# sarahappleby/VAMP

Measured on AMD Instinct MI355X. Metric: walker-steps/sec (log-posterior evals/sec), higher is better.
Workload: dtype f64

## Files before the change

vamp_amd/csrc/ff_moments.hpp:

```cpp
#pragma once
#include "voigt_math.hpp"

namespace vamp {

constexpr int FFM_NS = 14, FFM_NQ = 27, FFM_QROW = 28;
constexpr int FFM_S = 4 * FFM_QROW;
constexpr int FFM_TILE = FFM_S + 4 * FFM_NS;
constexpr int FFM_C0 = 0 * FFM_QROW + FFM_NQ;
constexpr int FFM_RC = 1 * FFM_QROW + FFM_NQ;
constexpr int FFM_RQ = 2 * FFM_QROW + FFM_NQ;

constexpr double FFM_ULPS = 8.0;
constexpr double FFM_BOUND = 256.0 / 1099511627776.0;
constexpr double FFM_RMAX = 512.0;
VAMP_DEV bool ff_moments_ok(double root_c0, double root_q0, double amax) {
    return fma(amax, root_q0, root_c0) <= FFM_RMAX;
}
VAMP_DEV bool ff_moments_try(double root_c0, double root_q0) {
    return ff_moments_ok(root_c0, root_q0, 0.0) && root_c0 + root_c0 <= FFM_RMAX;
}

}
```

vamp_amd/csrc/vamp_hip.hip:

```cpp
#include <hip/hip_runtime.h>
#include <dlfcn.h>

#include <algorithm>
#include <atomic>
#include <chrono>
#include <cmath>
#include <cstdint>
#include <cstdio>
#include <cstdlib>
#include <cstring>
#include <new>
#include <string>
#include <vector>

#include "../../include/vamp_hip.h"
#include "abi_state.hpp"
#include "draws.hpp"
#include "host_plan.hpp"
#include "map_search.hpp"
#include "voigt_math.hpp"
#include "ff_predicates.hpp"
#include "ff_moments.hpp"

#ifndef VAMP_EARLY_LOADS
#define VAMP_EARLY_LOADS 1
#endif
#ifndef VAMP_BLEND_PASS_LINES
#define VAMP_BLEND_PASS_LINES 4
#endif
#ifndef VAMP_MID_MIN_K
#define VAMP_MID_MIN_K 3
#endif
#ifndef VAMP_MID_MIN_P
#define VAMP_MID_MIN_P 96
#endif
#ifndef VAMP_X_PREFETCH
#define VAMP_X_PREFETCH 0
#endif

#ifndef VAMP_MIN_WAVES
#define VAMP_MIN_WAVES 3
#endif
#ifndef VAMP_EARLY_LNP
#define VAMP_EARLY_LNP 1
#endif
#ifndef VAMP_SR_EARLY
#define VAMP_SR_EARLY 0
#endif
#ifndef VAMP_XCD_MAP
#define VAMP_XCD_MAP 0
#endif
#ifndef VAMP_WIDE_NODES
#define VAMP_WIDE_NODES 1
#endif
#ifndef VAMP_LPT
#define VAMP_LPT 1
#endif
#ifndef VAMP_FLUX_EXP_DROP
#define VAMP_FLUX_EXP_DROP 2
#endif
#ifndef VAMP_FF_R2_M4
#define VAMP_FF_R2_M4 100.0
#define VAMP_FF_R2_M3 300.0
#define VAMP_FF_R2_M2 2000.0
#endif
#ifndef VAMP_F32_FAR_CORE
#define VAMP_F32_FAR_CORE 1
#endif
#ifndef VAMP_CORE_FASTPATH
#define VAMP_CORE_FASTPATH 1
#endif
#ifndef VAMP_MID_NODES
#define VAMP_MID_NODES 1
#endif
#ifndef VAMP_MID_Z2
#define VAMP_MID_Z2 30.25
#endif
#ifndef VAMP_WIDE_MAX
#define VAMP_WIDE_MAX 0.75
#endif
#ifndef VAMP_F32_LEAN_STAGE
#define VAMP_F32_LEAN_STAGE 1
#endif
#ifndef VAMP_TILE_MOMENTS
#define VAMP_TILE_MOMENTS 1
#endif
namespace {

constexpr int KMAX = 16;
constexpr int KMAX_ALL = VAMP_MAX_COMPONENTS;
static_assert(KMAX_ALL >= KMAX && KMAX_ALL < 64, "lane k stages line k; one spare lane for sd");
constexpr int WAVES_PER_BLOCK = 4;
constexpr long long PACK_MIN_WALKERS = 16384;
constexpr int RES_MAX_MOVERS = 128;
#ifndef VAMP_RES_WAVES
#define VAMP_RES_WAVES 8
#endif
constexpr int RES_MAX_WAVES = VAMP_RES_WAVES;
constexpr int BLOCK = 64 * WAVES_PER_BLOCK;
constexpr int DMAX = 4 * KMAX_ALL + 1;
#ifndef VAMP_SPLIT_MAX_WALKERS
#define VAMP_SPLIT_MAX_WALKERS (1ll << 62)
#endif
constexpr long long SPLIT_MAX_WALKERS = VAMP_SPLIT_MAX_WALKERS;

constexpr double C_LIGHT = 2.98e8;
constexpr double SIGMA0 = 0.0263;
constexpr double SQRT_LN2 = 0.83255461115769775635;
constexpr double SQRT_PI = 1.77245385090551602730;
constexpr double FWHM_PER_SIGMA = 2.35482004503094938202;
constexpr double NEG_INF = -__builtin_huge_val();

using vamp::RegionDev;

struct LineRec {
    double c;
    double s;
    double y;
    double amp;
    double pole;
    double hy;
    double xcap;
    double w8, w25;
    double wmid;
};

#ifndef VAMP_PARTS
#define VAMP_PARTS 4
#endif
constexpr int PARTS = VAMP_PARTS;
template <int KCAP, bool OWN_DTAB> struct WalkerLds;
#ifdef VAMP_STAMPS
__device__ unsigned long long g_stamps[2 * 8192];
__device__ unsigned int g_stamp_n;
#define VAMP_STAMP(tag)                                                                          \
    do {                                                                                         \
        if (blockIdx.x == 0 && threadIdx.x == 0) {                                               \
            const unsigned int n_ = g_stamp_n;                                                   \
            if (n_ < 8192) { g_stamps[2 * n_] = (tag); g_stamps[2 * n_ + 1] = __builtin_amdgcn_s_memtime(); g_stamp_n = n_ + 1; } \
        }                                                                                        \
    } while (0)
#define VAMP_STAMP_AFTER(tag, v) do { asm volatile("" :: "v"(v)); VAMP_STAMP(tag); } while (0)
#else
#define VAMP_STAMP(tag) do {} while (0)
#define VAMP_STAMP_AFTER(tag, v) do {} while (0)
#endif
#ifndef VAMP_SPLIT_WAVES
#define VAMP_SPLIT_WAVES 4
#endif
#ifndef VAMP_SPLIT_WAVES_F32
#define VAMP_SPLIT_WAVES_F32 4
#endif
#ifndef VAMP_F32_TABLES
#define VAMP_F32_TABLES 1
#endif
template <int LPW_, int KCAP_, bool TAIL_, int WPB_, bool SPLIT_ = false, bool TABS_ = SPLIT_, bool FF_ = (LPW_ == 64)>
struct Pack {
    static constexpr int LPW = LPW_, KCAP = KCAP_, SUBS = 64 / LPW_;
    static constexpr bool TAIL = TAIL_;
    static constexpr bool SPLIT = SPLIT_;
    static constexpr bool TABS = TABS_;
    static constexpr bool FF = FF_;
    static constexpr int WPB = WPB_;
    static constexpr int THREADS = 64 * WPB_;
    static constexpr int WALKERS_PER_BLOCK = SPLIT_ ? 1 : WPB_ * SUBS;
    static constexpr int LINES_PER_PASS = (SPLIT_ && TABS_ && !FF_ && WPB_ == 1) ? VAMP_BLEND_PASS_LINES : 0;
    static constexpr int TAB_LINES = LINES_PER_PASS > 0 ? LINES_PER_PASS : KCAP_;
    static constexpr bool DTAB_IN_TABLES = SPLIT_ && TABS_ && FF_;
// ... 552 lines not shown
}
template <class real>
__device__ __forceinline__ void ff_series(TileScratch& Sx, const double* __restrict__ dct, int lane, double fs) {
    if (lane < FF_NODES) Sx.coef[lane] = fs;
    __builtin_amdgcn_wave_barrier();
    const double2* mrow = reinterpret_cast<const double2*>(dct) + (lane < FF_ROWS ? lane : FF_ROWS - 1);
    const double2* fv = reinterpret_cast<const double2*>(Sx.coef);
    double a0 = 0.0, a1 = 0.0;
#pragma unroll
    for (int n2 = 0; n2 < FF_NODES / 2; ++n2) {
        const double2 m = mrow[n2 * FF_ROWS], f2 = fv[n2];
        a0 = fma(m.x, f2.x, a0);
        a1 = fma(m.y, f2.y, a1);
    }
    __builtin_amdgcn_wave_barrier();
    if (lane < FF_ROWS) reinterpret_cast<real*>(Sx.coef)[lane] = (real)(a0 + a1);
    __builtin_amdgcn_wave_barrier();
}
template <class LDS, bool GUARD = true>
__device__ __forceinline__ double ff_node_sums(const LDS& L, const unsigned char* farlist, const double* __restrict__ dct,
                                               int lane_, int nfar, double mid, double half, double fs_wide = 0.0) {
    int lane = lane_;
    asm volatile("" : "+v"(lane));
    const int node = lane & (FF_NODES - 1), grp = lane >> 4;
    const double tnode = dct[FF_MAT + node];
    __builtin_amdgcn_wave_barrier();
    const double xnode = fma(half, tnode, mid);
    double Xn[4], yn[4], an[4];
#pragma unroll
    for (int t = 0; t < 4; ++t) {
        const int q = 4 * t + grp;
        const unsigned kf = nfar > 0 ? farlist[q < nfar ? q : nfar - 1] : 0u;
        const LineRec& ln = *reinterpret_cast<const LineRec*>(reinterpret_cast<const char*>(L.line) + __umul24(kf, (unsigned)sizeof(LineRec)));
        Xn[t] = fabs(xnode - ln.c) * ln.s;
        yn[t] = ln.y;
        an[t] = q < nfar ? ln.amp : 0.0;
    }
    double fs = 0.0;
    if (nfar > 0) {
        const double Xa[2] = {Xn[0], Xn[1]}, ya[2] = {yn[0], yn[1]};
        double Ha[2];
        ff_eval2<GUARD>(Xa, ya, Ha, dct + FF_EXP);
        fs = fma(an[0], Ha[0], an[1] * Ha[1]);
    }
    if (nfar > 8) {
        const double Xb[2] = {Xn[2], Xn[3]}, yb[2] = {yn[2], yn[3]};
        double Hb[2];
        ff_eval2<GUARD>(Xb, yb, Hb, dct + FF_EXP);
        fs += fma(an[2], Hb[0], an[3] * Hb[1]);
    }
    fs += fs_wide;
    fs += __hiloint2double(__builtin_amdgcn_ds_bpermute((lane ^ 16) << 2, __double2hiint(fs)),
                           __builtin_amdgcn_ds_bpermute((lane ^ 16) << 2, __double2loint(fs)));
    fs += __hiloint2double(__builtin_amdgcn_ds_bpermute((lane ^ 32) << 2, __double2hiint(fs)),
                           __builtin_amdgcn_ds_bpermute((lane ^ 32) << 2, __double2loint(fs)));
    return fs;
}
template <class LDS, bool GUARD = true>
__device__ __forceinline__ void ff_coefficients(const LDS& L, TileScratch& Sx, const unsigned char* farlist, const double* __restrict__ dct,
                                                int lane, int nfar, double mid, double half, double fs_wide = 0.0) {
    ff_series<double>(Sx, dct, lane, ff_node_sums<LDS, GUARD>(L, farlist, dct, lane, nfar, mid, half, fs_wide));
}
__device__ __forceinline__ void ff_moment_chi(TileScratch& Sx, const double* __restrict__ dct, const double* __restrict__ mt, int lane,
                                              double a, double& chi) {
    const int row = lane < FF_ROWS ? lane : FF_ROWS - 1;
    const int q = row / (FF_DEG + 1), j = row - q * (FF_DEG + 1);
    ff_series<double>(Sx, dct, lane, a);
    const double* Qw = mt + q * vamp::FFM_QROW + j;
    double Qv[FF_DEG + 1];
#pragma unroll
    for (int l = 0; l <= FF_DEG; ++l) Qv[l] = Qw[l];
    const double Sv = mt[vamp::FFM_S + row], c0 = mt[vamp::FFM_C0];
    const double* bq = Sx.coef + q * (FF_DEG + 1);
    double acc0 = Sv + Sv, acc1 = 0.0;
#pragma unroll
    for (int l = 0; l <= FF_DEG; l += 2) {
        acc0 = fma(bq[l], Qv[l], acc0);
        acc1 = fma(bq[l + 1], Qv[l + 1], acc1);
    }
    const double term = Sx.coef[row] * (acc0 + acc1);
    chi += lane < FF_ROWS ? term : lane == FF_ROWS ? c0 : 0.0;
    __builtin_amdgcn_wave_barrier();
}
template <class LDS>
__device__ __forceinline__ double ff_wide_nodes(const LDS& L, const unsigned char* widelist, const double* __restrict__ dct, const double* tab,
                                                int lane, int nwide, double mid, double half) {
    const int node = lane & (FF_NODES - 1), grp = lane >> 4;
    const double xnode = fma(half, dct[FF_MAT + node], mid);
    double fs = 0.0;
    for (int t = 0; 4 * t < nwide; ++t) {
        const int q = 4 * t + grp;
        const int k = widelist[q < nwide ? q : nwide - 1];
        const LineRec& ln = L.line[k];
        const double X = fabs(xnode - ln.c) * ln.s, r2 = fma(X, X, ln.y * ln.y);
        double H;
        if (r2 < vamp::R2_CORE) {
            H = table_eval(tab + k * vamp::TAB_LINE, X);
        } else {
            H = vamp::voigt_jfrac<6>(X, ln.y, r2);
            if (ln.y < vamp::Y_TINY) H += vamp::SQRT_PI * vamp::exp_neg_sq_tab(X, dct + FF_EXP);
        }
        fs = fma(q < nwide ? ln.amp : 0.0, H, fs);
    }
    return fs;
}
template <class real, int T>
__device__ __forceinline__ void ff_horner(const TileScratch& Sx, const real (&u)[T], bool up, real (&tau)[T]) {
    static_assert(T == 4, "one pixel per quarter of the tile");
    real acc[T];
    const real* cq[T];
#pragma unroll
    for (int t = 0; t < T; ++t) {
        const int q = up ? t : T - 1 - t;
        cq[t] = reinterpret_cast<const real*>(Sx.coef) + q * (FF_DEG + 1);
        acc[t] = cq[t][FF_DEG];
    }
#pragma unroll
    for (int j = FF_DEG - 1; j >= 0; --j) {
#pragma unroll
        for (int t = 0; t < T; ++t) acc[t] = fma(acc[t], u[t], cq[t][j]);
    }
#pragma unroll
    for (int t = 0; t < T; ++t) tau[t] += acc[t];
    __builtin_amdgcn_wave_barrier();
}

template <int MODE, class PK, bool TAB, bool WIDE = false, bool GUARD = true>
__device__ __forceinline__ void sweep_range_ff(const RegionDev& R, const typename PK::Lds& L, TileScratch& Sx, const double* __restrict__ dct,
                                               const double* __restrict__ x, const double* __restrict__ f,
                                               const double* __restrict__ wt, const double* __restrict__ ut,
                                               const double2* __restrict__ geo, int lane, int base0, int base1, int stride,
                                               double& chi, const double* tab, unsigned long long wide_all = 0ull,
                                               const double* __restrict__ mom = nullptr) {
    constexpr int T = TPIX;
    static_assert(PK::LPW == 64 && PK::KCAP <= 16, "far-field tiles: one walker per wavefront, <= 16 lines");
    const int K = R.K;
#if VAMP_X_PREFETCH
    double xn[T];
    if (base0 < base1) {
#pragma unroll
        for (int t = 0; t < T; ++t) xn[t] = x[base0 + 64 * t + lane];
    }
#endif
    for (int batch = base0; batch < base1; batch += FF_BATCH * stride) {
    unsigned long long farmasks, widemasks, zonemasks;
    ff_classify_batch<WIDE, false, TAB>(L, Sx, geo, K, lane, batch, base1, stride, (unsigned)wide_all, farmasks, widemasks, zonemasks);
#if VAMP_TILE_MOMENTS && !defined(VAMP_SKIP_FFNODES)
    {
        unsigned long long fm = farmasks, wm = widemasks;
#pragma unroll 1
        for (int j = 0; j < FF_BATCH; ++j, fm >>= KMAX, wm >>= KMAX) {
            const int base = batch + j * stride;
            if (base >= base1) break;
            const unsigned farmask = (unsigned)fm & 0xffffu, widemask = WIDE ? (unsigned)wm & 0xffffu : 0u;
            if ((~(farmask | widemask) & ((1u << K) - 1u)) != 0u) continue;
            const double* mt = mom + (base >> 8) * vamp::FFM_TILE;
            const double root_c0 = mt[vamp::FFM_RC], root_q0 = mt[vamp::FFM_RQ];
            if (!vamp::ff_moments_try(root_c0, root_q0)) continue;
            const double2 tg = geo[base >> 8];
            const double mid = tg.x, half = fabs(tg.y);
            const int nfar = __builtin_popcount(farmask), nwide = __builtin_popcount(widemask);
            const int ln = lane_here();
            double fs_wide = 0.0;
            if constexpr (WIDE) {
                if (nwide > 0) fs_wide = ff_wide_nodes<typename PK::Lds>(L, Sx.widelist[j], dct, tab, ln, nwide, mid, half);
            }
            const double fs = ff_node_sums<typename PK::Lds, GUARD>(L, Sx.farlist[j], dct, ln, nfar, mid, half, fs_wide);
            int eoff = FF_EXP;
            asm volatile("" : "+s"(eoff));
            const double a = -vamp::expm1_taylor_tab(-fs, dct + eoff);
            const double amax = row16_max(fabs(a));
            if (!__builtin_amdgcn_readfirstlane((int)vamp::ff_moments_ok(root_c0, root_q0, amax))) continue;
            ff_moment_chi(Sx, dct, mt, ln, a, chi);
            const unsigned long long field = 0xffffull << (KMAX * j);
            farmasks |= field;
            widemasks |= field;
        }
    }
#endif
#pragma unroll 1
    for (int j = 0; j < FF_BATCH; ++j, farmasks >>= KMAX, widemasks >>= KMAX, zonemasks >>= KMAX) {
        const int base = batch + j * stride;
        if (base >= base1) break;
        double xi[T], tau[T];
#if VAMP_X_PREFETCH
#pragma unroll
        for (int t = 0; t < T; ++t) {
            xi[t] = xn[t];
            tau[t] = 0.0;
        }
        {
            const int nb = base + stride < base1 ? base + stride : base;
#pragma unroll
            for (int t = 0; t < T; ++t) xn[t] = x[nb + 64 * t + lane];
        }
#else
#pragma unroll
        for (int t = 0; t < T; ++t) {
            xi[t] = x[base + 64 * t + lane];
            tau[t] = 0.0;
        }
#endif
        if ((unsigned)farmasks & (unsigned)widemasks & 0xffffu) continue;
        const double2 tg = geo[base >> 8];
        const double mid = tg.x, half = fabs(tg.y);
        const bool up = __double2hiint(tg.y) >= 0;
        const unsigned farmask = (unsigned)farmasks & 0xffffu;
        const int nfar = __builtin_popcount(farmask);
        const unsigned widemask = WIDE ? (unsigned)widemasks & 0xffffu : 0u;
        const int nwide = __builtin_popcount(widemask);
#ifndef VAMP_SKIP_NEAR
        for (unsigned near = ~(farmask | widemask) & ((1u << K) - 1u); near; near &= near - 1u) {
            const int k = __builtin_ctz(near);
            const LineRec ln = L.line[k];
            double X[T], H[T];
#pragma unroll
            for (int t = 0; t < T; ++t) X[t] = fabs(xi[t] - ln.c) * ln.s;
            if (TAB && (((unsigned)zonemasks >> k) & 1u)) {
#pragma unroll
                for (int t = 0; t < T; ++t) H[t] = table_eval(tab + k * vamp::TAB_LINE, X[t]);
            } else {
                tile_voigt<T, TAB>(ln, dtab_row<PK>(L, k), X, H, TAB ? tab + k * vamp::TAB_LINE : nullptr, dct + FF_EXP);
            }
#pragma unroll
            for (int t = 0; t < T; ++t) tau[t] = fma(ln.amp, H[t], tau[t]);
        }
#endif
        double fi[T], wi[T];
        if (nfar + nwide > 0) {
            double u[T];
#pragma unroll
            for (int t = 0; t < T; ++t) u[t] = ut[base + 64 * t + lane];
#ifndef VAMP_SKIP_FFNODES
            double fs_wide = 0.0;
            if constexpr (WIDE) {
                if (nwide > 0) {
                    fs_wide = ff_wide_nodes<typename PK::Lds>(L, Sx.widelist[j], dct, tab, lane, nwide, mid, half);
                }
            }
            ff_coefficients<typename PK::Lds, GUARD>(L, Sx, Sx.farlist[j], dct, lane, nfar, mid, half, fs_wide);
#endif
#if VAMP_EARLY_LOADS
#pragma unroll
            for (int t = 0; t < T; ++t) {
                fi[t] = f[base + 64 * t + lane];
                wi[t] = wt[base + 64 * t + lane];
            }
            __builtin_amdgcn_sched_barrier(0);
#endif
#ifndef VAMP_SKIP_CLENSHAW
            ff_horner<double, T>(Sx, u, up, tau);
#endif
        } else {
#if VAMP_EARLY_LOADS
#pragma unroll
            for (int t = 0; t < T; ++t) {
// ... 214 lines not shown
            tau[t] = 0.0f;
        }
        const double2 tg = geo[base >> 8];
        const double mid = tg.x, half = fabs(tg.y);
        const bool up = __double2hiint(tg.y) >= 0;
        const unsigned farmask = (unsigned)farmasks & 0xffffu;
        const int nfar = __builtin_popcount(farmask);
#ifndef VAMP_SKIP_NEAR
        for (unsigned near = ~farmask & ((1u << K) - 1u); near; near &= near - 1u) {
            const int k = __builtin_ctz(near);
            const float c = L.linef[k][0], sc = L.linef[k][1], y = L.linef[k][2], a = L.linef[k][3];
            float X[T], H[T];
#pragma unroll
            for (int t = 0; t < T; ++t) X[t] = fabsf(xi[t] - c) * sc;
            if constexpr (TAB32) tile_w4_tab<T>(y, X, H, tab32 + k * vamp::TAB32_LINE);
            else tile_w4<T>(y, X, H);
#pragma unroll
            for (int t = 0; t < T; ++t) tau[t] = fmaf(a, H[t], tau[t]);
        }
#endif
        if (nfar > 0) {
            float u[T];
#pragma unroll
            for (int t = 0; t < T; ++t) u[t] = ut[base + 64 * t + lane];
#ifndef VAMP_SKIP_FFNODES
            ff32_coefficients<typename PK::Lds>(L, Sx, Sx.farlist[j], reinterpret_cast<const float*>(dct), lane, nfar, mid, half);
#endif
#ifndef VAMP_SKIP_CLENSHAW
            ff32_horner<T>(Sx, u, up, tau);
#endif
        }
#pragma unroll
        for (int t = 0; t < T; ++t) {
            const int i = base + 64 * t + lane;
#ifdef VAMP_SKIP_EXP
            const float m = 1.0f - tau[t];
#else
            const float m = __expf(-tau[t]);
#endif
            const float r = (f[i] - m) * wt[i];
            chi += (double)r * (double)r;
        }
    }
    }
}

struct PixPtrs {
    const double* x; const double* f; const double* wt;
    const float* xf; const float* ff; const float* wtf;
    const double* u; const float* uf; const double2* geo;
    const double* mom;
};

template <bool F32>
__global__ __launch_bounds__(64 * TPIX) void k_tile_tables(const RegionDev* __restrict__ regions, const double* __restrict__ x,
                                                           const float* __restrict__ xf, double* __restrict__ u, float* __restrict__ uf,
                                                           double2* __restrict__ geo, const double* __restrict__ f = nullptr,
                                                           const double* __restrict__ wt = nullptr, double* __restrict__ mom = nullptr) {
    const RegionDev& R = regions[blockIdx.y];
    const int base = (int)blockIdx.x * (64 * TPIX), i = base + (int)threadIdx.x;
    if (i >= R.P) return;
    const long long g = R.pix_off + i;
    if (base + 64 * TPIX > R.P) {
        if constexpr (F32) uf[g] = 0.0f;
        else u[g] = 0.0;
        return;
    }
    const long long g0 = R.pix_off + base, g1 = g0 + 64 * TPIX - 1;
    const double x_lo = F32 ? (double)xf[g0] : x[g0], x_hi = F32 ? (double)xf[g1] : x[g1];
    const double mid = 0.5 * (x_lo + x_hi), half = 0.5 * fabs(x_hi - x_lo);
    const bool up = x_hi > x_lo;
    const int t = (int)threadIdx.x >> 6, q = up ? t : TPIX - 1 - t;
    double ug = 0.0;
    if constexpr (F32) {
        const float hf = (float)half, mf = (float)mid;
        const float scale = 4.0f * __builtin_amdgcn_rcpf(hf);
        uf[g] = (xf[g] - fmaf(hf, 0.5f * q - 0.75f, mf)) * scale;
    } else {
        const double scale = 4.0 * vamp::rcp_nr(half);
        ug = (x[g] - fma(half, 0.5 * q - 0.75, mid)) * scale;
        u[g] = ug;
    }
    if (threadIdx.x == 0) geo[g0 >> 8] = make_double2(mid, up ? half : -half);
#if VAMP_TILE_MOMENTS
    if constexpr (!F32) {
        __shared__ double part[TPIX][2];
        double* mt = mom + (g0 >> 8) * vamp::FFM_TILE;
        const int lane = (int)threadIdx.x & 63;
        const double w2 = wt[g] * wt[g], d = f[g] - 1.0, w2d = w2 * d;
        double pw = 1.0;
        for (int n = 0; n < vamp::FFM_NQ; ++n) {
            const double sq = wave_sum<64>(w2 * pw);
            if (lane == 0) mt[q * vamp::FFM_QROW + n] = sq;
            if (n == 0 && lane == 0) part[q][0] = sq;
            if (n < vamp::FFM_NS) {
                const double ss = wave_sum<64>(w2d * pw);
                if (lane == 0) mt[vamp::FFM_S + q * vamp::FFM_NS + n] = ss;
            }
            pw *= ug;
        }
        const double c0 = wave_sum<64>(w2d * d);
        if (lane == 0) part[q][1] = c0;
        __syncthreads();
        if (threadIdx.x == 0) {
            const double q0 = (part[0][0] + part[1][0]) + (part[2][0] + part[3][0]);
            const double C0 = (part[0][1] + part[1][1]) + (part[2][1] + part[3][1]);
            mt[vamp::FFM_C0] = C0;
            mt[vamp::FFM_RC] = sqrt(C0);
            mt[vamp::FFM_RQ] = sqrt(q0);
            mt[3 * vamp::FFM_QROW + vamp::FFM_NQ] = 0.0;
        }
    }
#endif
}

template <bool F32, int MODE, class PK, bool TAB = use_tables<F32, MODE, PK>()>
__device__ __forceinline__ void sweep_class(const RegionDev& R, const typename PK::Lds& L, TileScratch& Sx, const double* __restrict__ dct,
                                            const PixPtrs& px, int lane, int base0, int full, int stride, bool tail, double& chi,
                                            const double* tab) {
    constexpr int TPIX = pixels_per_lane<PK>();
    if constexpr (F32) {
        const float* x = px.xf + R.pix_off; const float* f = px.ff + R.pix_off; const float* wt = px.wtf + R.pix_off;
        if constexpr (VAMP_FARFIELD && PK::FF && MODE != VAMP_GAUSS3 && TPIX == 4)
            sweep_range_f32_ff<MODE, PK, use_tables32<F32, MODE, PK>()>(R, L, Sx, dct, x, f, wt, px.uf + R.pix_off, px.geo + (R.pix_off >> 8),
                                                                        lane, base0, full, stride, chi, reinterpret_cast<const float*>(tab));
        else if (TPIX > 1) sweep_range_f32<MODE, PK, TPIX>(R, L, x, f, wt, lane, base0, full, stride, chi);
        if constexpr (PK::TAIL || TPIX == 1)
            if (tail) {
                const int from = TPIX > 1 ? full : 0;
                if constexpr (!PK::FF && TPIX > 1) {
                    const int nt = (R.P - from + PK::LPW - 1) / PK::LPW;
                    if constexpr (TPIX >= 4) { if (nt == 4) sweep_range_f32<MODE, PK, 4>(R, L, x, f, wt, lane, from, from + 1, 1 << 28, chi); }
                    if constexpr (TPIX >= 3) { if (nt == 3) sweep_range_f32<MODE, PK, 3>(R, L, x, f, wt, lane, from, from + 1, 1 << 28, chi); }
                    if (nt == 2) sweep_range_f32<MODE, PK, 2>(R, L, x, f, wt, lane, from, from + 1, 1 << 28, chi);
                    else if (nt == 1) sweep_range_f32<MODE, PK, 1>(R, L, x, f, wt, lane, from, from + 1, 1 << 28, chi);
                } else {
                    sweep_range_f32<MODE, PK, 1>(R, L, x, f, wt, lane, from, R.P, PK::LPW, chi);
                }
            }
    } else {
        const double* x = px.x + R.pix_off; const double* f = px.f + R.pix_off; const double* wt = px.wt + R.pix_off;
        if constexpr (VAMP_FARFIELD && PK::FF && MODE != VAMP_GAUSS3 && TPIX == 4) {
            const double* ut = px.u + R.pix_off;
            const double2* geo = px.geo + (R.pix_off >> 8);
            const double* mom = VAMP_TILE_MOMENTS ? px.mom + (R.pix_off >> 8) * vamp::FFM_TILE : nullptr;
            const int flags = __builtin_amdgcn_readfirstlane((int)(__double_as_longlong(L.theta[4 * PK::KCAP + 2]) & 0x3ffff));
            const bool guard = (flags >> 16) != 0;
            if constexpr (VAMP_WIDE_NODES && TAB) {
                const unsigned long long wide_all = (unsigned long long)(flags & 0xffff);
                if (VAMP_MID_NODES || wide_all) {
                    if (guard) sweep_range_ff<MODE, PK, TAB, true, true>(R, L, Sx, dct, x, f, wt, ut, geo, lane, base0, full, stride, chi, tab, wide_all, mom);
                    else sweep_range_ff<MODE, PK, TAB, true, false>(R, L, Sx, dct, x, f, wt, ut, geo, lane, base0, full, stride, chi, tab, wide_all, mom);
                } else {
                    if (guard) sweep_range_ff<MODE, PK, TAB, false, true>(R, L, Sx, dct, x, f, wt, ut, geo, lane, base0, full, stride, chi, tab, 0ull, mom);
                    else sweep_range_ff<MODE, PK, TAB, false, false>(R, L, Sx, dct, x, f, wt, ut, geo, lane, base0, full, stride, chi, tab, 0ull, mom);
                }
            } else {
                if (guard) sweep_range_ff<MODE, PK, TAB, false, true>(R, L, Sx, dct, x, f, wt, ut, geo, lane, base0, full, stride, chi, tab, 0ull, mom);
                else sweep_range_ff<MODE, PK, TAB, false, false>(R, L, Sx, dct, x, f, wt, ut, geo, lane, base0, full, stride, chi, tab, 0ull, mom);
            }
        } else if (TPIX > 1) sweep_range<MODE, PK, TPIX, TAB>(R, L, x, f, wt, lane, base0, full, stride, chi, tab);
        if constexpr (PK::TAIL || TPIX == 1)
            if (tail) {
                const int from = TPIX > 1 ? full : 0;
                if constexpr (!PK::FF && TPIX > 1) {
                    const int nt = (R.P - from + PK::LPW - 1) / PK::LPW;
                    if constexpr (TPIX >= 4) { if (nt == 4) sweep_range<MODE, PK, 4, TAB>(R, L, x, f, wt, lane, from, from + 1, 1 << 28, chi, tab); }
                    if constexpr (TPIX >= 3) { if (nt == 3) sweep_range<MODE, PK, 3, TAB>(R, L, x, f, wt, lane, from, from + 1, 1 << 28, chi, tab); }
                    if (nt == 2) sweep_range<MODE, PK, 2, TAB>(R, L, x, f, wt, lane, from, from + 1, 1 << 28, chi, tab);
                    else if (nt == 1) sweep_range<MODE, PK, 1, TAB>(R, L, x, f, wt, lane, from, from + 1, 1 << 28, chi, tab);
                } else {
                    sweep_range<MODE, PK, 1, TAB>(R, L, x, f, wt, lane, from, R.P, PK::LPW, chi, tab);
                }
            }
    }
}

template <int MODE, class PK, int T>
__device__ __forceinline__ void blend_chunk(const RegionDev& R, const typename PK::Lds& L, const double* __restrict__ x, int lane,
                                            int base, int k0, int kn, const double* tab, double (&tau)[4]) {
    double xi[T];
#pragma unroll
    for (int t = 0; t < T; ++t) {
        const int i = base + 64 * t + lane;
        xi[t] = x[i < R.P ? i : R.P - 1];
    }
    for (int kk = 0; kk < kn; ++kk) {
        const LineRec ln = L.line[k0 + kk];
        double X[T], H[T];
#pragma unroll
        for (int t = 0; t < T; ++t) X[t] = fabs(xi[t] - ln.c) * ln.s;
        tile_voigt<T, true>(ln, L.dtab[k0 + kk], X, H, tab + kk * vamp::TAB_LINE);
#pragma unroll
        for (int t = 0; t < T; ++t) tau[t] = fma(ln.amp, H[t], tau[t]);
    }
}
template <int MODE, class PK>
__device__ __forceinline__ void blend_chunk_n(const RegionDev& R, const typename PK::Lds& L, const double* __restrict__ x, int lane,
                                              int base, int tn, int k0, int kn, const double* tab, double (&tau)[4]) {
    if (tn >= 4) blend_chunk<MODE, PK, 4>(R, L, x, lane, base, k0, kn, tab, tau);
    else if (tn == 3) blend_chunk<MODE, PK, 3>(R, L, x, lane, base, k0, kn, tab, tau);
    else if (tn == 2) blend_chunk<MODE, PK, 2>(R, L, x, lane, base, k0, kn, tab, tau);
    else if (tn == 1) blend_chunk<MODE, PK, 1>(R, L, x, lane, base, k0, kn, tab, tau);
}
constexpr int BLEND_MAX_PIXELS = 512;
template <int MODE, class PK>
__device__ __forceinline__ double sweep_blend_passes(const RegionDev& R, const typename PK::Lds& L, const PixPtrs& px, int lane,
                                                     double* tab) {
    static_assert(PK::WPB == 1 && PK::LPW == 64, "one wavefront per walker");
    constexpr int LP = PK::LINES_PER_PASS;
    const double* __restrict__ x = px.x + R.pix_off;
    const double* __restrict__ f = px.f + R.pix_off;
    const double* __restrict__ wt = px.wt + R.pix_off;
    const int P = R.P, K = R.K;
    const int nt = (P + 63) >> 6;
    const int tn0 = nt < 4 ? nt : 4, tn1 = nt - tn0;
    double tau0[4] = {0.0, 0.0, 0.0, 0.0}, tau1[4] = {0.0, 0.0, 0.0, 0.0};
    for (int k0 = 0; k0 < K; k0 += LP) {
        const int kn = K - k0 < LP ? K - k0 : LP;
        for (int e = lane; e < kn * vamp::TAB_NI; e += 64) {
            const int kk = e / vamp::TAB_NI, i = e % vamp::TAB_NI, k = k0 + kk;
            vamp::taylor_table_row(i, L.line[k].y, L.dtab[k], L.line[k].pole, L.line[k].hy, tab + kk * vamp::TAB_LINE + i * vamp::TAB_NT);
        }
        group_barrier<PK>();
        blend_chunk_n<MODE, PK>(R, L, x, lane, 0, tn0, k0, kn, tab, tau0);
        if (tn1 > 0) blend_chunk_n<MODE, PK>(R, L, x, lane, 256, tn1, k0, kn, tab, tau1);
        group_barrier<PK>();
    }
// ... 1316 lines not shown
    if (c->comm && c->exchange && c->shard_parts > 1)
        for (int p = 0; p < c->shard_parts; ++p) HIP_TRY(hipStreamWaitEvent(c->stream, c->ev_scatter[p], 0));
    return 0;
}

int free_comm(vamp_ctx* c) {
    if (c->rccl) {
        RcclApi* api = nullptr;
        if (rccl_api(&api) == 0) (void)api->CommDestroy(c->rccl);
        c->rccl = nullptr;
    }
    for (hipEvent_t e : c->ev_kernel) (void)hipEventDestroy(e);
    for (hipEvent_t e : c->ev_scatter) (void)hipEventDestroy(e);
    c->ev_kernel.clear();
    c->ev_scatter.clear();
    if (c->comm_stream) (void)hipStreamDestroy(c->comm_stream);
    c->comm_stream = nullptr;
    vamp::leave_comm(c);
    return 0;
}

}

extern "C" {

long long vampdbg_resident_plan(vamp_ctx* c, int max_classes, long long* rows) {
    if (!c || !rows || max_classes < 0) return fail(VAMP_ERR_ARG, "vampdbg_resident_plan: bad argument");
    if (!c->sampler_ready) return fail(VAMP_ERR_STATE, "vampdbg_resident_plan: call vamp_sampler_init first");
    const long long halfW = c->W / 2;
    const std::vector<LaunchClass>& classes = partition_for(c, halfW);
    for (size_t ci = 0; ci < classes.size() && (int)ci < max_classes; ++ci) {
        const LaunchClass& cl = classes[ci];
        const int shape = launch_shape(c, cl, halfW);
        const int nw = resident_waves_for(c, shape, halfW);
        long long lds = 0;
        VAMP_FOR_MODE_PK(c->f32, c->mode, shape, lds = resident_lds<F32, M, PK>(nw));
        long long* row = rows + 4 * ci;
        row[0] = cl.kind;
        row[1] = nw;
        row[2] = (long long)nw * (shape_walkers_per_block(shape) / shape_waves(shape));
        row[3] = lds;
    }
    return (long long)classes.size();
}

long long vampdbg_launch_plan(vamp_ctx* c, long long movers_per_region, int entry, int region, int max_classes, long long* rows) {
    if (!c || !rows || max_classes < 0 || entry < 0 || entry > 3 || movers_per_region < 1) return fail(VAMP_ERR_ARG, "vampdbg_launch_plan: bad argument");
    if (c->regions_h.empty()) return fail(VAMP_ERR_STATE, "vampdbg_launch_plan: call vamp_set_regions first");
    if (region >= c->n_regions || (entry == 2 && region < 0)) return fail(VAMP_ERR_ARG, "vampdbg_launch_plan: no such region");
    const long long per = entry == 3 ? MAP_MOVERS : movers_per_region;
    const std::vector<LaunchClass>& classes = partition_for(c, per);
    const std::vector<int>& class_of = class_of_for(c, per);
    long long n = 0;
    for (size_t ci = 0; ci < classes.size(); ++ci) {
        const LaunchClass& cl = classes[ci];
        if (region >= 0 && class_of[region] != (int)ci) continue;
        if (n < max_classes) {
            const int shape = launch_shape(c, cl, per);
            long long* row = rows + 5 * n;
            row[0] = cl.kind;
            row[1] = shape;
            row[2] = shape_walkers_per_block(shape);
            row[3] = shape_threads(shape);
            row[4] = (long long)cl.regions.size();
        }
        ++n;
    }
    return n;
}

long long vampdbg_tile_tables(vamp_ctx* c, double* u_out, float* uf_out, double* geo_out) {
    if (!c || !geo_out || !(c->f32 ? (void*)uf_out : (void*)u_out)) return fail(VAMP_ERR_ARG, "vampdbg_tile_tables: bad argument");
    if (c->regions_h.empty()) return fail(VAMP_ERR_STATE, "vampdbg_tile_tables: call vamp_set_regions first");
    if (!c->geo_d) return 0;
    const long long N = c->regions_h.back().pix_off + c->regions_h.back().P;
    const long long slots = N / (64 * TPIX) + 1;
    HIP_TRY(hipStreamSynchronize(c->stream));
    if (c->f32) HIP_TRY(hipMemcpy(uf_out, c->uf_d.get(), N * sizeof(float), hipMemcpyDeviceToHost));
    else HIP_TRY(hipMemcpy(u_out, c->u_d.get(), N * sizeof(double), hipMemcpyDeviceToHost));
    HIP_TRY(hipMemcpy(geo_out, c->geo_d.get(), slots * sizeof(double2), hipMemcpyDeviceToHost));
    return slots;
}

int vamp_version(void) { return VAMP_ABI_VERSION; }

const char* vamp_last_error(void) { return vamp::last_error().c_str(); }

int vamp_device_count(int* n) {
    if (int rc = vamp::check_device_count(n)) return rc;
    HIP_TRY(hipGetDeviceCount(n));
    return VAMP_OK;
}

int vamp_ctx_create(vamp_ctx** out, int device, int dtype, int wofz_kind) {
    if (int rc = vamp::check_ctx_create(out, dtype, wofz_kind)) return rc;
    int ndev = 0;
    HIP_TRY(hipGetDeviceCount(&ndev));
    if (int rc = vamp::check_device(device, ndev)) return rc;
    HIP_TRY(hipSetDevice(device));
    vamp_ctx* c = nullptr;
    if (int rc = vamp::new_ctx(&c, dtype)) return rc;
    c->device = device;
    c->wofz_kind = wofz_kind;
    hipError_t e = hipStreamCreateWithFlags(&c->own_stream, hipStreamNonBlocking);
    if (e != hipSuccess) {
        delete c;
        return fail(VAMP_ERR_HIP, std::string("hipStreamCreate: ") + hipGetErrorString(e));
    }
    c->stream = c->own_stream;
    if (const char* e = getenv("VAMP_CLASS_STREAMS")) c->concurrent_classes = std::atoi(e) != 0;
    if (const char* e = getenv("VAMP_RESIDENT")) c->opt_resident = std::max(0, std::min(2, std::atoi(e)));
    if (const char* e = getenv("VAMP_MAP_DEVICE")) c->opt_map_device = std::atoi(e) != 0;
    *out = c;
    return VAMP_OK;
}

int vamp_ctx_destroy(vamp_ctx* c) {
    if (!c) return VAMP_OK;
    (void)hipSetDevice(c->device);
    (void)hipStreamSynchronize(c->stream);
    if (c->comm_stream) (void)hipStreamSynchronize(c->comm_stream);
    free_comm(c);
    for (hipStream_t st : c->cls_stream) (void)hipStreamDestroy(st);
    for (hipEvent_t e : c->ev_join) (void)hipEventDestroy(e);
    if (c->ev_fork) (void)hipEventDestroy(c->ev_fork);
    if (c->own_stream) (void)hipStreamDestroy(c->own_stream);
    delete c;
    return VAMP_OK;
}

int vamp_ctx_set_stream(vamp_ctx* c, void* hip_stream) {
    if (int rc = vamp::need_ctx(c, "vamp_ctx_set_stream")) return rc;
    HIP_TRY(hipStreamSynchronize(c->stream));
    c->stream = hip_stream ? (hipStream_t)hip_stream : c->own_stream;
    return VAMP_OK;
}

int vamp_ctx_set_stream_default(vamp_ctx* c) {
    if (int rc = vamp::need_ctx(c, "vamp_ctx_set_stream_default")) return rc;
    HIP_TRY(hipStreamSynchronize(c->stream));
    c->stream = nullptr;
    return VAMP_OK;
}

int vamp_ctx_set_packing(vamp_ctx* c, int lanes_per_walker) { return vamp::set_packing(c, lanes_per_walker); }

int vamp_ctx_set_option(vamp_ctx* c, const char* name, int64_t value) {
    if (int rc = vamp::check_option(c, name)) return rc;
    const std::string key(name);
    if (key == "map_device") c->opt_map_device = value != 0;
    else if (key == "resident") c->opt_resident = value < 0 ? 0 : value > 2 ? 2 : (int)value;
    else c->concurrent_classes = value != 0;
    return VAMP_OK;
}

int vamp_ctx_synchronize(vamp_ctx* c) {
    if (int rc = vamp::need_ctx(c, "vamp_ctx_synchronize")) return rc;
    HIP_TRY(hipSetDevice(c->device));
    HIP_TRY(hipStreamSynchronize(c->stream));
    return VAMP_OK;
}

int vamp_set_regions(vamp_ctx* c, int n_regions, const int64_t* pix_off, const double* x, const double* flux,
                     const double* noise, const int32_t* n_comp, int mode, int sample_sd, int include_norm,
                     const double* bounds, const double* nbz) {
    if (int rc = vamp::check_set_regions(c, n_regions, pix_off, x, flux, noise, n_comp, mode, nbz)) return rc;
    HIP_TRY(hipSetDevice(c->device));
    HIP_TRY(hipStreamSynchronize(c->stream));
    reset_sampler(c);
    reset_regions(c);
    static_assert(KMAX == 16 && KMAX_ALL == 32 && PackSmall::KCAP == 8 && PackSmall2::KCAP == 2 && VAMP_MID_MIN_K == 3 &&
                  VAMP_MID_MIN_P == 96 && BLEND_MAX_PIXELS == 512 && 64 * TPIX == 256, "vamp::plan::Limits describes these shapes");
    if (int rc = vamp::build_regions(c, n_regions, pix_off, x, noise, n_comp, mode, sample_sd, include_norm, bounds, nbz, VAMP_F32_TABLES != 0))
        return rc;
    const std::vector<RegionDev>& R = c->regions_h;
    const long long N = pix_off[n_regions];
    const std::vector<double> wt = vamp::pixel_weights(N, noise, sample_sd);
    HIP_TRY(c->x_d.ensure(N));
    HIP_TRY(c->f_d.ensure(N));
    HIP_TRY(c->wt_d.ensure(N));
    HIP_TRY(hipMemcpy(c->x_d.get(), x, N * sizeof(double), hipMemcpyHostToDevice));
    HIP_TRY(hipMemcpy(c->f_d.get(), flux, N * sizeof(double), hipMemcpyHostToDevice));
    HIP_TRY(hipMemcpy(c->wt_d.get(), wt.data(), N * sizeof(double), hipMemcpyHostToDevice));
    if (c->f32) {
        std::vector<float> t(N);
        HIP_TRY(c->xf_d.ensure(N));
        HIP_TRY(c->ff_d.ensure(N));
        HIP_TRY(c->wtf_d.ensure(N));
        for (long long i = 0; i < N; ++i) t[i] = (float)x[i];
        HIP_TRY(hipMemcpy(c->xf_d.get(), t.data(), N * sizeof(float), hipMemcpyHostToDevice));
        for (long long i = 0; i < N; ++i) t[i] = (float)flux[i];
        HIP_TRY(hipMemcpy(c->ff_d.get(), t.data(), N * sizeof(float), hipMemcpyHostToDevice));
        for (long long i = 0; i < N; ++i) t[i] = (float)wt[i];
        HIP_TRY(hipMemcpy(c->wtf_d.get(), t.data(), N * sizeof(float), hipMemcpyHostToDevice));
    }
    HIP_TRY(c->regions_d.ensure(n_regions));
    HIP_TRY(hipMemcpy(c->regions_d.get(), R.data(), n_regions * sizeof(RegionDev), hipMemcpyHostToDevice));
    int max_tiles = 0;
    bool any_full = false;
    for (const RegionDev& d : R) {
        max_tiles = std::max(max_tiles, (d.P + 64 * TPIX - 1) / (64 * TPIX));
        any_full = any_full || d.P >= 64 * TPIX;
    }
    if (mode != VAMP_GAUSS3 && any_full) {
        if (c->f32) HIP_TRY(c->uf_d.ensure(N));
        else HIP_TRY(c->u_d.ensure(N));
        HIP_TRY(c->geo_d.ensure(N / (64 * TPIX) + 1));
        if (VAMP_TILE_MOMENTS && !c->f32) HIP_TRY(c->mom_d.ensure((N / (64 * TPIX) + 1) * vamp::FFM_TILE));
        VAMP_FOR_F32(c->f32, hipLaunchKernelGGL((k_tile_tables<F32>), dim3((unsigned)max_tiles, (unsigned)n_regions), dim3(64 * TPIX), 0,
                                                c->stream, c->regions_d.get(), c->x_d.get(), c->xf_d.get(), c->u_d.get(),
                                                c->uf_d.get(), c->geo_d.get(), c->f_d.get(), c->wt_d.get(), c->mom_d.get()));
        HIP_TRY(hipGetLastError());
        HIP_TRY(hipStreamSynchronize(c->stream));
    }
    for (int which = 0; which < 2; ++which) {
        const vamp::plan::ClassPlan& pl = which ? c->plan_small : c->plan;
        std::vector<LaunchClass>& part = which ? c->classes_small : c->classes;
        for (size_t k = 0; k < pl.kind.size(); ++k) part.push_back(LaunchClass{pl.kind[k], pl.regions[k]});
#if VAMP_LPT
        bool reordered = false;
        if (which == 1 || VAMP_LPT == 2)
            for (LaunchClass& cl : part) {
                std::vector<int> before = cl.regions;
                std::stable_sort(cl.regions.begin(), cl.regions.end(), [&](int a, int b) {
                    return (long long)R[a].K * R[a].P > (long long)R[b].K * R[b].P;
                });
                reordered = reordered || before != cl.regions;
            }
        if (part.size() > 1 || reordered)
#else
        if (part.size() > 1)
#endif
            for (LaunchClass& cl : part) {
                HIP_TRY(cl.list_d.ensure(cl.regions.size()));
                HIP_TRY(hipMemcpy(cl.list_d.get(), cl.regions.data(), cl.regions.size() * sizeof(int), hipMemcpyHostToDevice));
            }
    }
    c->n_regions = n_regions;
    c->n_pix = N;
    return VAMP_OK;
}

int vamp_set_region_ids(vamp_ctx* c, const int32_t* ids) {
    if (int rc = vamp::set_region_ids(c, ids)) return rc;
    HIP_TRY(hipSetDevice(c->device));
    HIP_TRY(hipStreamSynchronize(c->stream));
    HIP_TRY(hipMemcpy(c->regions_d.get(), c->regions_h.data(), c->n_regions * sizeof(RegionDev), hipMemcpyHostToDevice));
    return VAMP_OK;
}

int vamp_region_class(vamp_ctx* c, int region, int* kind, int* n_classes) { return vamp::region_class(c, region, kind, n_classes); }

int vamp_region_ndim(vamp_ctx* c, int region, int* ndim) { return vamp::region_ndim(c, region, ndim); }

namespace {
int launch_lnprob(vamp_ctx* c, int region, long long W, const double* th_d, double* lp_d, double* ch_d) {
    const bool all = region < 0;
    const long long per = lnprob_movers(W);
    const std::vector<LaunchClass>& classes = partition_for(c, per);
    const std::vector<int>& class_of = class_of_for(c, per);
    for (size_t ci = 0; ci < classes.size(); ++ci) {
        const LaunchClass& cl = classes[ci];
        if (!all && class_of[region] != (int)ci) continue;
        const int shape = launch_shape(c, cl, per);
        const long long per_block = shape_walkers_per_block(shape);
        const dim3 grid((unsigned)((W + per_block - 1) / per_block), all ? (unsigned)cl.regions.size() : 1u);
        const dim3 threads(shape_threads(shape));
        VAMP_FOR_MODE_PK(c->f32, c->mode, shape, hipLaunchKernelGGL((k_lnprob<F32, M, PK>), grid, threads, 0, c->stream, c->regions_d.get(), region,
                                                                c->pix(), W, th_d, lp_d, ch_d, (const int*)cl.list_d.get()));
        HIP_TRY(hipGetLastError());
    }
    return 0;
}

constexpr size_t PINNED_EVAL_BYTES = 1u << 20;
int lnprob_impl(vamp_ctx* c, int region, int64_t W, const double* theta, double* lnprob, double* chi2) {
    HIP_TRY(hipSetDevice(c->device));
    const bool all = region < 0;
    const long long dsum = all ? c->regions_h.back().d_before + c->regions_h.back().D : c->regions_h[region].D;
    const size_t nth = (size_t)W * dsum;
    const size_t nout = (size_t)W * (all ? c->n_regions : 1);
    if (nth * sizeof(double) <= PINNED_EVAL_BYTES) {
        HIP_TRY(c->pin_th.ensure(std::max(nth, (size_t)4096)));
        HIP_TRY(c->pin_out.ensure(std::max(2 * nout, (size_t)1024)));
        std::memcpy(c->pin_th.get(), theta, nth * sizeof(double));
        double* lp_h = c->pin_out.get();
        double* ch_h = chi2 ? lp_h + nout : nullptr;
        int rc = launch_lnprob(c, region, W, c->pin_th.get(), lp_h, ch_h);
        if (rc) return rc;
        HIP_TRY(hipStreamSynchronize(c->stream));
        std::memcpy(lnprob, lp_h, nout * sizeof(double));
// ... 444 lines not shown
```

Baseline: 12.85 million.

## Precompute tile moments in node (Lagrange) basis to skip series transform in chi

Adds a second tile-moment layout that stores the weighted Gram matrix of the 16 far-field node Lagrange interpolants, plus the data projection and constant term, for each tile. The per-step chi evaluation then contracts the node absorption values directly against this matrix. This skips the per-step Chebyshev series transform and the 27-wide quadratic-form dot. It also makes the moments zeroed before setup and adds a debug accessor. The setup kernel does more work and the record grows to 280 doubles, which could add memory traffic per tile.

```diff
diff --git a/vamp_amd/csrc/ff_moments.hpp b/vamp_amd/csrc/ff_moments.hpp
--- a/vamp_amd/csrc/ff_moments.hpp
+++ b/vamp_amd/csrc/ff_moments.hpp
@@ -10,6 +10,15 @@
 constexpr int FFM_RC = 1 * FFM_QROW + FFM_NQ;
 constexpr int FFM_RQ = 2 * FFM_QROW + FFM_NQ;
 
+constexpr int FFN_NODES = 16;
+constexpr int FFN_Q = 0;
+constexpr int FFN_S = FFN_NODES * FFN_NODES;
+constexpr int FFN_C0 = FFN_S + FFN_NODES;
+constexpr int FFN_RC = FFN_C0 + 1;
+constexpr int FFN_RQ = FFN_C0 + 2;
+constexpr int FFN_TILE = 280;
+static_assert(FFN_TILE >= FFN_RQ + 1 && FFN_TILE % 8 == 0, "the record fits, and a tile starts on a 64-byte line");
+
 constexpr double FFM_ULPS = 8.0;
 constexpr double FFM_BOUND = 256.0 / 1099511627776.0;
 constexpr double FFM_RMAX = 512.0;
diff --git a/vamp_amd/csrc/vamp_hip.hip b/vamp_amd/csrc/vamp_hip.hip
--- a/vamp_amd/csrc/vamp_hip.hip
+++ b/vamp_amd/csrc/vamp_hip.hip
@@ -83,7 +83,7 @@
 #define VAMP_F32_LEAN_STAGE 1
 #endif
 #ifndef VAMP_TILE_MOMENTS
-#define VAMP_TILE_MOMENTS 1
+#define VAMP_TILE_MOMENTS 2
 #endif
 namespace {
 
@@ -802,6 +802,24 @@
     chi += lane < FF_ROWS ? term : lane == FF_ROWS ? c0 : 0.0;
     __builtin_amdgcn_wave_barrier();
 }
+__device__ __forceinline__ void ff_moment_chi_nodes(TileScratch& Sx, const double* __restrict__ mt, int lane, double a, double c0, double& chi) {
+    static_assert(FF_NODES == vamp::FFN_NODES, "the record is laid out for the node stage's 16 nodes");
+    if (lane < FF_NODES) Sx.coef[lane] = a;
+    const int n = lane & (FF_NODES - 1), g4 = (lane >> 4) * 4;
+    const double2* Qr = reinterpret_cast<const double2*>(mt + vamp::FFN_Q + n * FF_NODES + g4);
+    const double2 q01 = Qr[0], q23 = Qr[1];
+    const double Sv = mt[vamp::FFN_S + n];
+    __builtin_amdgcn_wave_barrier();
+    const double2* av = reinterpret_cast<const double2*>(Sx.coef + g4);
+    const double2 a01 = av[0], a23 = av[1];
+    const double acc0 = fma(q01.x, a01.x, 0.5 * Sv), acc1 = q01.y * a01.y;
+    const double term = a * (fma(q23.x, a23.x, acc0) + fma(q23.y, a23.y, acc1));
+    chi += lane == 0 ? term + c0 : term;
+    __builtin_amdgcn_wave_barrier();
+}
+constexpr int MOM_TILE = VAMP_TILE_MOMENTS == 2 ? vamp::FFN_TILE : vamp::FFM_TILE;
+constexpr int MOM_RC = VAMP_TILE_MOMENTS == 2 ? vamp::FFN_RC : vamp::FFM_RC;
+constexpr int MOM_RQ = VAMP_TILE_MOMENTS == 2 ? vamp::FFN_RQ : vamp::FFM_RQ;
 template <class LDS>
 __device__ __forceinline__ double ff_wide_nodes(const LDS& L, const unsigned char* widelist, const double* __restrict__ dct, const double* tab,
                                                 int lane, int nwide, double mid, double half) {
@@ -874,8 +892,8 @@
             if (base >= base1) break;
             const unsigned farmask = (unsigned)fm & 0xffffu, widemask = WIDE ? (unsigned)wm & 0xffffu : 0u;
             if ((~(farmask | widemask) & ((1u << K) - 1u)) != 0u) continue;
-            const double* mt = mom + (base >> 8) * vamp::FFM_TILE;
-            const double root_c0 = mt[vamp::FFM_RC], root_q0 = mt[vamp::FFM_RQ];
+            const double* mt = mom + (base >> 8) * MOM_TILE;
+            const double root_c0 = mt[MOM_RC], root_q0 = mt[MOM_RQ];
             if (!vamp::ff_moments_try(root_c0, root_q0)) continue;
             const double2 tg = geo[base >> 8];
             const double mid = tg.x, half = fabs(tg.y);
@@ -891,7 +909,11 @@
             const double a = -vamp::expm1_taylor_tab(-fs, dct + eoff);
             const double amax = row16_max(fabs(a));
             if (!__builtin_amdgcn_readfirstlane((int)vamp::ff_moments_ok(root_c0, root_q0, amax))) continue;
+#if VAMP_TILE_MOMENTS == 2
+            ff_moment_chi_nodes(Sx, mt, ln, a, mt[vamp::FFN_C0], chi);
+#else
             ff_moment_chi(Sx, dct, mt, ln, a, chi);
+#endif
             const unsigned long long field = 0xffffull << (KMAX * j);
             farmasks |= field;
             widemasks |= field;
@@ -1272,7 +1294,59 @@
         u[g] = ug;
     }
     if (threadIdx.x == 0) geo[g0 >> 8] = make_double2(mid, up ? half : -half);
-#if VAMP_TILE_MOMENTS
+#if VAMP_TILE_MOMENTS == 2
+    if constexpr (!F32) {
+        constexpr int NN = vamp::FFN_NODES, NPIX = 64 * TPIX;
+        __shared__ double ell[NN][NPIX];
+        __shared__ double w2s[NPIX], w2ds[NPIX], part[TPIX][2];
+        const int p = (int)threadIdx.x;
+        const double tp = (x[g] - mid) / half;
+        double c[NN], den = 0.0;
+        int hit = -1;
+#pragma unroll
+        for (int n = 0; n < NN; ++n) {
+            const double tn = FF_M[FF_MAT + n], wn = sqrt((1.0 - tn) * (1.0 + tn)), diff = tp - tn;
+            if (diff == 0.0) hit = n;
+            c[n] = ((n & 1) ? -wn : wn) / diff;
+            den += c[n];
+        }
+#pragma unroll
+        for (int n = 0; n < NN; ++n) ell[n][p] = hit < 0 ? c[n] / den : (n == hit ? 1.0 : 0.0);
+        const double w2 = wt[g] * wt[g], d = f[g] - 1.0, w2d = w2 * d;
+        w2s[p] = w2;
+        w2ds[p] = w2d;
+        __syncthreads();
+        double* mt = mom + (g0 >> 8) * vamp::FFN_TILE;
+        const int n = p >> 4, m = p & (NN - 1);
+        double qa[8] = {0.0, 0.0, 0.0, 0.0, 0.0, 0.0, 0.0, 0.0}, sa[8] = {0.0, 0.0, 0.0, 0.0, 0.0, 0.0, 0.0, 0.0};
+        for (int i = 0; i < NPIX; i += 8) {
+#pragma unroll
+            for (int k = 0; k < 8; ++k) qa[k] = fma(w2s[i + k], ell[n][i + k] * ell[m][i + k], qa[k]);
+        }
+        mt[vamp::FFN_Q + p] = ((qa[0] + qa[1]) + (qa[2] + qa[3])) + ((qa[4] + qa[5]) + (qa[6] + qa[7]));
+        if (p < NN) {
+            for (int i = 0; i < NPIX; i += 8) {
+#pragma unroll
+                for (int k = 0; k < 8; ++k) sa[k] = fma(w2ds[i + k], ell[p][i + k], sa[k]);
+            }
+            mt[vamp::FFN_S + p] = ((sa[0] + sa[1]) + (sa[2] + sa[3])) + ((sa[4] + sa[5]) + (sa[6] + sa[7]));
+        }
+        const double cw = wave_sum<64>(w2d * d), qw = wave_sum<64>(w2);
+        if ((p & 63) == 0) {
+            part[p >> 6][0] = qw;
+            part[p >> 6][1] = cw;
+        }
+        __syncthreads();
+        if (p == 0) {
+            const double q0 = (part[0][0] + part[1][0]) + (part[2][0] + part[3][0]);
+            const double C0 = (part[0][1] + part[1][1]) + (part[2][1] + part[3][1]);
+            mt[vamp::FFN_C0] = C0;
+            mt[vamp::FFN_RC] = sqrt(C0);
+            mt[vamp::FFN_RQ] = sqrt(q0);
+        }
+        if (p > vamp::FFN_RQ - vamp::FFN_S && p < vamp::FFN_TILE - vamp::FFN_S) mt[vamp::FFN_S + p] = 0.0;
+    }
+#elif VAMP_TILE_MOMENTS
     if constexpr (!F32) {
         __shared__ double part[TPIX][2];
         double* mt = mom + (g0 >> 8) * vamp::FFM_TILE;
@@ -1333,7 +1407,7 @@
         if constexpr (VAMP_FARFIELD && PK::FF && MODE != VAMP_GAUSS3 && TPIX == 4) {
             const double* ut = px.u + R.pix_off;
             const double2* geo = px.geo + (R.pix_off >> 8);
-            const double* mom = VAMP_TILE_MOMENTS ? px.mom + (R.pix_off >> 8) * vamp::FFM_TILE : nullptr;
+            const double* mom = VAMP_TILE_MOMENTS ? px.mom + (R.pix_off >> 8) * MOM_TILE : nullptr;
             const int flags = __builtin_amdgcn_readfirstlane((int)(__double_as_longlong(L.theta[4 * PK::KCAP + 2]) & 0x3ffff));
             const bool guard = (flags >> 16) != 0;
             if constexpr (VAMP_WIDE_NODES && TAB) {
@@ -2816,6 +2890,17 @@
     return slots;
 }
 
+long long vampdbg_tile_moments(vamp_ctx* c, double* out) {
+    if (!c) return fail(VAMP_ERR_ARG, "vampdbg_tile_moments: bad argument");
+    if (c->regions_h.empty()) return fail(VAMP_ERR_STATE, "vampdbg_tile_moments: call vamp_set_regions first");
+    if (!VAMP_TILE_MOMENTS || c->f32 || !c->geo_d || !c->mom_d) return 0;
+    const long long N = c->regions_h.back().pix_off + c->regions_h.back().P;
+    const long long slots = N / (64 * TPIX) + 1;
+    HIP_TRY(hipStreamSynchronize(c->stream));
+    if (out) HIP_TRY(hipMemcpy(out, c->mom_d.get(), slots * MOM_TILE * sizeof(double), hipMemcpyDeviceToHost));
+    return MOM_TILE;
+}
+
 int vamp_version(void) { return VAMP_ABI_VERSION; }
 
 const char* vamp_last_error(void) { return vamp::last_error().c_str(); }
@@ -2940,7 +3025,10 @@
         if (c->f32) HIP_TRY(c->uf_d.ensure(N));
         else HIP_TRY(c->u_d.ensure(N));
         HIP_TRY(c->geo_d.ensure(N / (64 * TPIX) + 1));
-        if (VAMP_TILE_MOMENTS && !c->f32) HIP_TRY(c->mom_d.ensure((N / (64 * TPIX) + 1) * vamp::FFM_TILE));
+        if (VAMP_TILE_MOMENTS && !c->f32) {
+            HIP_TRY(c->mom_d.ensure((N / (64 * TPIX) + 1) * MOM_TILE));
+            HIP_TRY(hipMemsetAsync(c->mom_d.get(), 0, (N / (64 * TPIX) + 1) * MOM_TILE * sizeof(double), c->stream));
+        }
         VAMP_FOR_F32(c->f32, hipLaunchKernelGGL((k_tile_tables<F32>), dim3((unsigned)max_tiles, (unsigned)n_regions), dim3(64 * TPIX), 0,
                                                 c->stream, c->regions_d.get(), c->x_d.get(), c->xf_d.get(), c->u_d.get(),
                                                 c->uf_d.get(), c->geo_d.get(), c->f_d.get(), c->wt_d.get(), c->mom_d.get()));
```

Measured after the change: 13.52 million (median of 6 runs). 5.2% higher.
